# PM25/Information-Retrieval-with-Contrastive-Learning

Hardware: AMD Instinct MI355X
Metric: query-doc pairs/sec (train) + queries/sec @ top-k over N docs, 1/2/4/8 GPU (higher is better)
Workload: dtype bf16

## Files before the change

include/irc.h:

```cpp
#ifndef IRC_H_
#define IRC_H_

#include <stdint.h>

#ifdef __cplusplus
extern "C" {
#endif

typedef void* irc_stream_t;

#define IRC_OK 0
#define IRC_E_INVALID 1001
#define IRC_E_WORKSPACE 1002
#define IRC_E_LAUNCH 1003

const char* irc_last_error(void);
int irc_abi_version(void);

int64_t irc_scan_topk_workspace(int64_t Q, int64_t N, int64_t D, int64_t k);
int irc_scan_topk(const void* queries, const void* docs, int64_t Q, int64_t N, int64_t D,
                  int64_t k, int64_t doc_offset, void* workspace, int64_t workspace_bytes,
                  float* out_score, int64_t* out_idx, irc_stream_t stream);

int irc_scan_topk_many(const void* const* queries, int64_t batches, const void* docs, int64_t Q,
// ... 61 lines not shown
int irc_quantize_fp8(int in_dtype, const void* x, int64_t n, float scale, void* out,
                     irc_stream_t stream);

int irc_gemm(int in_dtype, int out_dtype, int a_layout, int b_layout, int epilogue, int64_t M,
             int64_t N, int64_t K, float alpha, const void* A, int64_t lda, int64_t strideA,
             const void* B, int64_t ldb, int64_t strideB, const float* bias, int64_t strideBias,
             const void* R, int64_t ldr, int64_t strideR, void* C, int64_t ldc, int64_t strideC,
             int accumulate, int64_t batch, void* workspace, int64_t workspace_bytes,
             irc_stream_t stream);
int64_t irc_gemm_workspace(int in_dtype, int out_dtype, int epilogue, int64_t M, int64_t N,
                           int64_t K, int64_t batch);
int irc_gemm_ex(int in_dtype, int out_dtype, int a_layout, int b_layout, int epilogue, int64_t M,
                int64_t N, int64_t K, float alpha, const void* A, int64_t lda, int64_t strideA,
                const void* B, int64_t ldb, int64_t strideB, const float* bias, int64_t strideBias,
                const void* R, int64_t ldr, int64_t strideR, void* C, int64_t ldc, int64_t strideC,
                int accumulate, int64_t batch, void* workspace, int64_t workspace_bytes,
                int64_t max_blocks, irc_stream_t stream);
int64_t irc_gemm_workspace_ex(int in_dtype, int out_dtype, int epilogue, int64_t M, int64_t N,
                              int64_t K, int64_t batch, int64_t max_blocks);
int irc_gemm_set_persistent(int mode);
int irc_gemm_set_big_ring(int on);
int irc_gemm_ln(int epilogue, int64_t M, int64_t N, int64_t K, const void* A, int64_t lda,
                const void* B, int64_t ldb, const float* bias, const void* R, int64_t ldr,
                void* C, int64_t ldc, const float* ln_stats, int ln_nt, const float* ln_gamma,
                const float* ln_beta, float ln_eps, int64_t ln_h, const float* fold_colsum,
                float* stats_out, int* stats_nt_out, irc_stream_t stream);
int irc_gemm_set_big_mf16(int on);
int irc_gemm_set_big_dma(int on);
int irc_gemm_big_dma_fits(int64_t M, int64_t N, int64_t K, int64_t lda, int64_t ldb);
int irc_gemm_set_l2_touch(int mode);
int64_t irc_gemm_l2_touch_map(int operand, int64_t tiles_m, int64_t tiles_n, int64_t window,
                              int64_t lines, int64_t nk, int64_t dist, int32_t* count,
                              int32_t* owner, int32_t* sharers);

int irc_gemm_set_pp(int on);

int irc_embed_ln(int dtype, const int64_t* ids, const void* word, const void* pos,
                 const void* type0, const float* gamma, const float* beta, void* y, int64_t rows,
                 int64_t L, int64_t H, float eps, irc_stream_t stream);
int irc_layernorm(int dtype, const void* x, void* y, const float* gamma, const float* beta,
                  int64_t rows, int64_t H, float eps, irc_stream_t stream);
int irc_attention(int dtype, const void* qkv, const int64_t* mask, void* ctx, int64_t B,
                  int64_t L, int64_t H, int64_t heads, irc_stream_t stream);
int irc_qkv_attention(int64_t M, int64_t H, int64_t heads, int64_t L, const void* x, int64_t ldx,
                      const void* wqkv_perm, const float* bias_perm, const int64_t* mask,
                      void* ctx, int64_t ldc, irc_stream_t stream);

int64_t irc_layernorm_bwd_workspace(int64_t rows, int64_t H);
int irc_layernorm_bwd(int dtype, int dy_dtype, const void* dy, const void* x, const float* gamma,
                      void* dx, float* dgamma, float* dbeta, float* partial,
                      int64_t partial_floats, int64_t rows, int64_t H, float eps, int64_t bcast_L,
                      float dy_scale, int accumulate, irc_stream_t stream);
int irc_attention_bwd(int dtype, const void* qkv, const int64_t* mask, const void* ctx,
                      const void* dctx, void* dqkv, int64_t B, int64_t L, int64_t H,
                      int64_t heads, irc_stream_t stream);
int irc_embed_sum(int dtype, const int64_t* ids, const void* word, const void* pos,
                  const void* type0, float* y, int64_t rows, int64_t L, int64_t H,
                  irc_stream_t stream);
int irc_embed_bwd(int dtype, const void* dx, const int64_t* ids, float* dword, float* dpos,
                  float* dtype0, float* workspace, int64_t ws_floats, int64_t B, int64_t L,
                  int64_t H, int64_t pad_id, irc_stream_t stream);

int irc_lstm_fwd(int dtype, const float* xp, const void* whh, void* hout, float* gsave,
                 float* csave, void* hprev, int64_t B, int64_t L, int64_t H, int64_t ndir,
                 irc_stream_t stream);
int irc_lstm_bwd(int dtype, const float* dy, const void* whh, const float* gsave,
// ... 159 lines not shown
```

information-retrieval-with-contrastive-learning_amd/csrc/gemm.hip:

```cpp
#include "gemm_epi.h"
#include "gemm_pp.h"

#include <algorithm>
#include <atomic>
#include <type_traits>

#ifndef IRC_GEMM_GROUP_M
#define IRC_GEMM_GROUP_M 0
#endif

namespace irc {
namespace gemm {

enum Layout { ROW = 0, COL = 1 };

constexpr int BM = 128, BN = 128, NT = 256;

template <typename T>
struct TT;
template <>
struct TT<unsigned short> {
  static constexpr int BK = 32;
  static constexpr int VEC = 8;
  static constexpr int PITCH = BK * 2 + 16;
// ... 424 lines not shown
  constexpr int CH = ROWS * 4;
  static_assert(CH % NT == 0, "whole passes");
#pragma unroll
  for (int i = 0; i < CH / NT; ++i) {
    const int p = (i * NW + wave) * 64 + lane;
    const int row = p >> 2;
    const int c = (p & 3) ^ ((row >> 2) & 3);
    int gr = r0 + row;
    gr = gr < nrows ? gr : nrows - 1;
    glds16(X + (int64_t)gr * ld + k0 + c * 8, lds_tile + (i * NW + wave) * 1024);
  }
}

#ifdef IRC_BIG_STAMPS
__device__ uint64_t big_stamps[64][5][2];
#define BSTAMP(kt, i)                                                                      \
  do {                                                                                     \
    __builtin_amdgcn_sched_barrier(0);                                                     \
    if (blockIdx.x == 0 && threadIdx.x == 0 && (kt) < 64) {                               \
      uint64_t c_, r_;                                                                     \
      asm volatile("s_memtime %0\n\ts_memrealtime %1\n\ts_waitcnt lgkmcnt(0)"            \
                   : "=s"(c_), "=s"(r_)::"memory");                                        \
      *(volatile uint64_t*)&big_stamps[(kt)][(i)][0] = c_;                                 \
      *(volatile uint64_t*)&big_stamps[(kt)][(i)][1] = r_;                                 \
    }                                                                                      \
    __builtin_amdgcn_sched_barrier(0);                                                     \
  } while (0)
#else
#define BSTAMP(kt, i) \
  do {                \
  } while (0)
#endif

template <int WNB>
__device__ __forceinline__ void mainloop_mf16(const unsigned short* A, int64_t lda,
                                              const unsigned short* B, int64_t ldb, int m0,
                                              int n0, int M, int N, int K, char* lds, int wave,
                                              int lane, f32x4 (&acc4)[8][2 * WNB], bool dma,
                                              const Touch tch, int ls = 0, int sh = 6) {
  constexpr int BN = 128 * WNB;
  constexpr int A_BYTES = BM * ROW_BYTES, STAGE = A_BYTES + BN * ROW_BYTES;
  const int wm = wave >> 2, wn = wave & 3;
  const int nk = K / BK;
  const int a_rows = ls == 0 ? 64 : ls;
  const int a_row0 = ls == 0 ? m0 : (m0 >> sh) * ls;
  const bool buf = dma && (ls == 0 || sh == 6) && a_row0 + (BM / 64) * a_rows <= M && n0 + BN <= N;
  const __amdgpu_buffer_rsrc_t ra = buffer_rsrc(A, (uint32_t)(((int64_t)(M - 1) * lda + K) * 2));
  const __amdgpu_buffer_rsrc_t rb = buffer_rsrc(B, (uint32_t)(((int64_t)(N - 1) * ldb + K) * 2));
  const uint32_t a_pass = (uint32_t)a_rows * (uint32_t)lda * 2u, b_pass = 128u * (uint32_t)ldb;
  const uint32_t a_tile = (uint32_t)a_row0 * (uint32_t)lda * 2u;
  const uint32_t b_tile = (uint32_t)n0 * (uint32_t)ldb * 2u;
  uint32_t a_lane = 0, b_lane = 0;
  uint32_t ta_lane = 0, tb_lane = 0, sink = 0;
  uint64_t ta_mask = 0, tb_mask = 0;
  int touch_nk = 0;
  if (buf && (tch.a_n | tch.b_n) != 0) {
    touch_nk = nk - TOUCH_D;
    const int t = wave * 64 + lane;
    const int ar = tch.a_lo + t;
    const int arow = ls == 0 ? ar : (ar >> 6) * ls + min(ar & 63, ls - 1);
    ta_lane = (uint32_t)arow * (uint32_t)lda * 2u;
    tb_lane = (uint32_t)(tch.b_lo + t) * (uint32_t)ldb * 2u;
    ta_mask = __builtin_amdgcn_ballot_w64(t < tch.a_n);
    tb_mask = __builtin_amdgcn_ballot_w64(t < tch.b_n);
  }
  if (buf) {
    a_lane = dma_lane_off(lda, wave, lane, ls);
// ... 18 lines not shown
    BSTAMP(kt, 0);
    char* nxt = lds + (cur ^ 1) * STAGE;
    if (more && buf) {
      const uint32_t kb = (uint32_t)(kt + 1) * ROW_BYTES;
      stage_buf<BM>(ra, a_lane, a_tile + kb, a_pass, nxt, wave);
      stage_buf<BN>(rb, b_lane, b_tile + kb, b_pass, nxt + A_BYTES, wave);
      if (kt < touch_nk) {
        const uint32_t kd = (uint32_t)(kt + TOUCH_D) * ROW_BYTES;
        if (ta_mask != 0) touch_dword(sink, ra, ta_lane, a_tile + kd, ta_mask);
        if (tb_mask != 0) touch_dword(sink, rb, tb_lane, b_tile + kd, tb_mask);
      }
    } else if (more) {
      int ln = lane;
      asm volatile("" : "+v"(ln));
      stage<BM>(A, lda, m0, M, (kt + 1) * BK, nxt, wave, ln, ls, sh);
      stage<BN>(B, ldb, n0, N, (kt + 1) * BK, nxt + A_BYTES, wave, ln);
    }
    BSTAMP(kt, 1);
    const char* la = lds + cur * STAGE;
    const char* lb = la + A_BYTES;
#pragma unroll
    for (int s2 = 0; s2 < 2; ++s2) {
      const int coff = (((4 * s2 + q4) ^ key) * 16);
      bf16x8 fa[8];
#pragma unroll
      for (int i = 0; i < 8; ++i)
        fa[i] = *reinterpret_cast<const bf16x8*>(la + (wm * 128 + i * 16 + l16) * 128 + coff);
#pragma unroll
      for (int j = 0; j < 2 * WNB; ++j) {
        const bf16x8 fb =
            *reinterpret_cast<const bf16x8*>(lb + (wn * 32 * WNB + j * 16 + l16) * 128 + coff);
#pragma unroll
        for (int i = 0; i < 8; ++i)
          acc4[i][j] = __builtin_amdgcn_mfma_f32_16x16x32_bf16(fa[i], fb, acc4[i][j], 0, 0, 0);
      }
    }
    BSTAMP(kt, 2);
    wait_vmcnt<0>();
    BSTAMP(kt, 3);
    __syncthreads();
    BSTAMP(kt, 4);
  }
  touch_done(sink);
}
}

inline std::atomic<int>& big_ring_mode() {
  static std::atomic<int> on{0};
  return on;
}
inline bool big_ring() { return big_ring_mode().load(std::memory_order_relaxed) != 0; }

inline std::atomic<int>& big_mf16_mode() {
  static std::atomic<int> on{1};
  return on;
}
inline bool big_mf16() { return big_mf16_mode().load(std::memory_order_relaxed) != 0; }

inline std::atomic<int>& big_dma_mode() {
  static std::atomic<int> on{1};
  return on;
}
inline int big_dma_flag(int64_t M, int64_t N, int64_t K, int64_t lda, int64_t ldb) {
  return big_dma_mode().load(std::memory_order_relaxed) != 0 && big::dma_fits(M, K, lda) &&
         big::dma_fits(N, K, ldb);
}

constexpr int L2_TOUCH_MAX_TILES_N = 2;
inline std::atomic<int>& l2_touch_mode() {
  static std::atomic<int> mode{[] {
    const char* e = getenv("IRC_GEMM_L2_TOUCH");
    return e && e[0] >= '0' && e[0] <= '2' ? e[0] - '0' : 1;
  }()};
  return mode;
}
inline int l2_touch_flag(int big_dma, int group_m, int64_t tiles_n) {
  const int mode = l2_touch_mode().load(std::memory_order_relaxed);
  if (mode == 0 || !big_dma || group_m > 1) return 0;
  if (mode == 1 && tiles_n > L2_TOUCH_MAX_TILES_N) return 0;
  const int cus = gpp::cu_count();
  return cus >= 8 ? cus / 8 : 32;
}

template <int EPI, int WNB>
__device__ __forceinline__ void big_epilogue_bf16(const Args& g, const f32x4 (&acc4)[8][2 * WNB],
                                                  char* lds, unsigned short* C,
                                                  const unsigned short* R, const float* bias,
                                                  int m0, int n0, int wave, int lane) {
  constexpr int BN = 128 * WNB, WCOLS = 32 * WNB, PITCH = WCOLS + 8;
  constexpr int CPR = WCOLS / 8;
  constexpr int NCH = 32 * CPR / 64;
  constexpr int NB = CPR == 12 ? 3 : 1;
  constexpr int RSTEP = 64 * NB / CPR;
  static_assert(64 * NB % CPR == 0 && NCH % NB == 0, "the chunk map repeats every NB iterations");
  constexpr bool READS_R = EPI == EPI_BIAS_RESID || EPI == EPI_RESID || EPI == EPI_DGELU;
  constexpr bool USES_R = READS_R || EPI == EPI_BIAS_GELU_SAVE;
  const int wm = wave >> 2, wn = wave & 3;
  float* st = reinterpret_cast<float*>(lds) + wave * (32 * PITCH);
// ... 98 lines not shown
        if constexpr (READS_R) {
          if (i < 3) load_r(i + 1, it);
        }
      }
    } else {
#pragma unroll
      for (int it = 0; it < NCH; ++it) {
        const int c = it * 64 + lane;
        const int rl = c / CPR, c8 = (c % CPR) * 8;
        const int row = rbase + rl, col = cbase + c8;
        if (row >= g.M || col >= g.N) continue;
        const f32x4 v0 = *reinterpret_cast<const f32x4*>(&st[rl * PITCH + c8]);
        const f32x4 v1 = *reinterpret_cast<const f32x4*>(&st[rl * PITCH + c8 + 4]);
        const unsigned short* rp = USES_R ? R + (int64_t)row * g.ldr + col : nullptr;
        u16x8 rr = {};
        if constexpr (READS_R) rr = *reinterpret_cast<const u16x8*>(rp);
        const u16x8 o = finish(v0, v1, rr, rp);
#ifdef IRC_PP_DIAG_NOSTORE
        if (o[0] == 0x7fc1 && o[7] == 0x7fc3)
#endif
        *reinterpret_cast<u16x8*>(C + (int64_t)row * g.ldc + col) = o;
      }
    }
    __builtin_amdgcn_wave_barrier();
    asm volatile("s_waitcnt lgkmcnt(0)" ::: "memory");
  }
  };
  if (fast)
    passes(std::true_type{});
  else
    passes(std::false_type{});
}

template <typename TO, int EPI, int WNB, bool RING = false, bool MF16 = false, bool LN = false>
__global__ __launch_bounds__(big::NT, 1) void gemm_big_kernel(Args g) {
  static_assert(!(RING && MF16), "the 16x16x32 form is 2-slot only");
  static_assert(!LN || (MF16 && sizeof(TO) == 2), "the LayerNorm fold: 16x16x32 form, bf16 C");
  using big::BK;
  using big::NT;
  using big::NW;
  constexpr int BM = big::BM, BN = 128 * WNB;
  constexpr int A_BYTES = BM * big::ROW_BYTES, B_BYTES = BN * big::ROW_BYTES;
  constexpr int STAGE = A_BYTES + B_BYTES;
  __shared__ __attribute__((aligned(1024))) char lds[2 * STAGE];
  const int tiles_m = (g.M + BM - 1) / BM;
  const int tiles_n = (g.N + BN - 1) / BN;
  const int ntiles = tiles_m * tiles_n;
  int bid = blockIdx.x;
  {
    const int q = ntiles / 8, r = ntiles % 8, x = bid % 8;
    bid = (x < r ? x * (q + 1) : r * (q + 1) + (x - r) * q) + bid / 8;
  }
  int tm, tn;
  grouped_tile(bid, tiles_m, tiles_n, g.group_m, tm, tn);
  const int batch = blockIdx.y;
  const unsigned short* A = reinterpret_cast<const unsigned short*>(g.A) + batch * g.sA;
  const unsigned short* B = reinterpret_cast<const unsigned short*>(g.B) + batch * g.sB;
  TO* C = reinterpret_cast<TO*>(g.C) + batch * g.sC;
  const int m0 = tm * BM, n0 = tn * BN;
  const int lane = threadIdx.x & 63;
  const int wave = __builtin_amdgcn_readfirstlane(threadIdx.x >> 6);
  const int wm = wave >> 2, wn = wave & 3;
  const int h = lane >> 5, r32 = lane & 31;

  f32x16 acc[4][WNB];
  f32x4 acc4[8][2 * WNB];
#pragma unroll
  for (int i = 0; i < 4; ++i)
#pragma unroll
    for (int j = 0; j < WNB; ++j) acc[i][j] = (f32x16)0.0f;
// ... 18 lines not shown
    const int sw4 = (r32 >> 2) & 3;
    for (int kt = 0; kt < nk; ++kt) {
      const int after = nk - 1 - kt;
      if (after >= 2) wait_vmcnt<2 * PPT>();
      else if (after == 1) wait_vmcnt<PPT>();
      else wait_vmcnt<0>();
      wg_barrier();
      if (kt + 3 < nk) {
        char* nxt = lds + ((kt + 3) & 3) * STG4;
        big::stage4<BM>(A, g.lda, m0, g.M, (kt + 3) * BK4, nxt, wave, lane);
        big::stage4<BN>(B, g.ldb, n0, g.N, (kt + 3) * BK4, nxt + A4, wave, lane);
      }
      const char* la = lds + (kt & 3) * STG4;
      const char* lb = la + A4;
#pragma unroll
      for (int kk = 0; kk < BK4 / 16; ++kk) {
        const int coff = ((2 * kk + h) ^ sw4) * 16;
        bf16x8 fa[4], fb[WNB];
#pragma unroll
        for (int i = 0; i < 4; ++i)
          fa[i] = *reinterpret_cast<const bf16x8*>(la + (wm * 128 + i * 32 + r32) * ROW4 + coff);
#pragma unroll
        for (int j = 0; j < WNB; ++j)
          fb[j] = *reinterpret_cast<const bf16x8*>(lb + (wn * 32 * WNB + j * 32 + r32) * ROW4 + coff);
#pragma unroll
        for (int i = 0; i < 4; ++i)
#pragma unroll
          for (int j = 0; j < WNB; ++j)
            acc[i][j] = __builtin_amdgcn_mfma_f32_32x32x16_bf16(fa[i], fb[j], acc[i][j], 0, 0, 0);
      }
    }
    __syncthreads();
  } else if constexpr (MF16) {
    big::mainloop_mf16<WNB>(A, g.lda, B, g.ldb, m0, n0, g.M, g.N, g.K, lds, wave, lane, acc4,
                            g.big_dma != 0,
                            big::touch_lines(g.l2_touch, tiles_m, tiles_n, tm, tn, BM, BN));
  } else {
  const int nk = g.K / BK;
  big::stage<BM>(A, g.lda, m0, g.M, 0, lds, wave, lane);
  big::stage<BN>(B, g.ldb, n0, g.N, 0, lds + A_BYTES, wave, lane);
  wait_vmcnt<0>();
  __syncthreads();
  const int swz = big::chunk_key(r32);
  for (int kt = 0; kt < nk; ++kt) {
    const int cur = kt & 1;
#ifdef IRC_PP_DIAG_NODMA
    const bool more = kt + 1 < nk && kt < 0;
#else
    const bool more = kt + 1 < nk;
#endif
    if (more) {
      char* nxt = lds + (cur ^ 1) * STAGE;
      big::stage<BM>(A, g.lda, m0, g.M, (kt + 1) * BK, nxt, wave, lane);
      big::stage<BN>(B, g.ldb, n0, g.N, (kt + 1) * BK, nxt + A_BYTES, wave, lane);
    }
    const char* la = lds + cur * STAGE;
    const char* lb = la + A_BYTES;
#pragma unroll
    for (int kk = 0; kk < BK / 16; ++kk) {
      const int coff = (((2 * kk + h) ^ swz) * 16);
      bf16x8 fa[4], fb[WNB];
#pragma unroll
      for (int i = 0; i < 4; ++i)
        fa[i] = *reinterpret_cast<const bf16x8*>(la + (wm * 128 + i * 32 + r32) * 128 + coff);
#pragma unroll
      for (int j = 0; j < WNB; ++j)
        fb[j] = *reinterpret_cast<const bf16x8*>(lb + (wn * 32 * WNB + j * 32 + r32) * 128 + coff);
#pragma unroll
      for (int i = 0; i < 4; ++i)
// ... 567 lines not shown
          for (int e = 0; e < 16; ++e) {
            const int i = 32 * ib + (e & 3) + 8 * (e >> 2) + 4 * h;
            if (i < g.L) out[(int64_t)i * g.ldc + 32 * db + r32] = f32_to_bf16(o[db][e]);
          }
      }
    }
    if (hf == 0) __syncthreads();
  }
}

inline int big_wnb(const Args& g, int batch, int la, int lb) {
  if (la != ROW || lb != ROW || !g.vec_a || !g.vec_b) return 0;
  if (g.K % big::BK != 0 || g.K == 0) return 0;
  const int wnb = g.N % 384 == 0 ? 3 : 2;
  const int64_t tiles = (int64_t)((g.M + 255) / 256) * ((g.N + 128 * wnb - 1) / (128 * wnb)) * batch;
  return tiles >= 128 ? wnb : 0;
}

template <typename TO, int EPI, bool LN = false>
static int launch_big(const Args& g0, int batch, int wnb, hipStream_t st) {
  Args g = g0;
  g.big_dma = big_dma_flag(g.M, g.N, g.K, g.lda, g.ldb);
  const int bn = 128 * wnb;
  g.l2_touch = l2_touch_flag(g.big_dma, g.group_m, (g.N + bn - 1) / bn);
  const int tiles = ((g.M + big::BM - 1) / big::BM) * ((g.N + bn - 1) / bn);
  prof_begin(st);
  const bool ring = big_ring() && g.K % big::BK4 == 0;
  if constexpr (LN) {
    if (wnb == 3)
      hipLaunchKernelGGL((gemm_big_kernel<TO, EPI, 3, false, true, true>), dim3(tiles, batch), dim3(big::NT), 0, st, g);
    else
      hipLaunchKernelGGL((gemm_big_kernel<TO, EPI, 2, false, true, true>), dim3(tiles, batch), dim3(big::NT), 0, st, g);
  } else if (big_mf16() && !ring) {
    if (wnb == 3)
      hipLaunchKernelGGL((gemm_big_kernel<TO, EPI, 3, false, true>), dim3(tiles, batch), dim3(big::NT), 0, st, g);
    else
      hipLaunchKernelGGL((gemm_big_kernel<TO, EPI, 2, false, true>), dim3(tiles, batch), dim3(big::NT), 0, st, g);
  } else if (wnb == 3 && ring)
    hipLaunchKernelGGL((gemm_big_kernel<TO, EPI, 3, true>), dim3(tiles, batch), dim3(big::NT), 0, st, g);
  else if (wnb == 3)
    hipLaunchKernelGGL((gemm_big_kernel<TO, EPI, 3>), dim3(tiles, batch), dim3(big::NT), 0, st, g);
  else if (ring)
    hipLaunchKernelGGL((gemm_big_kernel<TO, EPI, 2, true>), dim3(tiles, batch), dim3(big::NT), 0, st, g);
  else
    hipLaunchKernelGGL((gemm_big_kernel<TO, EPI, 2>), dim3(tiles, batch), dim3(big::NT), 0, st, g);
  prof_end("gemm_bf16", st, 2.0 * g.M * g.N * g.K * batch);
  prof_work("gemm_bf16_bytes", gemm_alg_bytes(sizeof(TO) == 4, EPI, g.accumulate, g.M, g.N, g.K,
                                               batch));
  return check_launch("gemm_big_kernel");
}

template <typename TI, typename TO, int LA, int LB, int EPI>
static int launch(const Args& g0, int batch, int splits, hipStream_t st) {
  if constexpr (sizeof(TI) == 2) {
    if (splits == 1) {
      const int wnb = big_wnb(g0, batch, LA, LB);
      if (wnb) return launch_big<TO, EPI>(g0, batch, wnb, st);
    }
  }
  Args g = g0;
  const int tiles = ((g.M + BM - 1) / BM) * ((g.N + BN - 1) / BN);
  constexpr int bk = TT<TI>::BK;
  g.kchunk = splits > 1 ? ((g.K + splits - 1) / splits + bk - 1) / bk * bk : (g.K > 0 ? g.K : 1);
  prof_begin(st);
  hipLaunchKernelGGL((gemm_kernel<TI, TO, LA, LB, EPI>), dim3(tiles, batch, splits), dim3(NT), 0,
                     st, g);
  if (splits > 1) {
// ... 201 lines not shown
extern "C" int64_t irc_gemm_l2_touch_map(int operand, int64_t tiles_m, int64_t tiles_n,
                                         int64_t window, int64_t lines, int64_t nk,
                                         int64_t dist, int32_t* count, int32_t* owner,
                                         int32_t* sharers) {
  using namespace irc::gemm;
  if ((operand != 0 && operand != 1) || tiles_m < 1 || tiles_n < 1 || window < 1 || lines < 1 ||
      lines > big::NT || nk < 1 || dist < 1 || tiles_m > (1 << 20) || tiles_n > (1 << 20) ||
      window > (1 << 20) || !count || !owner)
    return -1;
  for (int64_t i = 0; i < nk * lines; ++i) count[i] = 0, owner[i] = -1;
  int s_a, rank_a, s_b, rank_b;
  big::touch_share((int)tiles_m, (int)tiles_n, (int)window, 0, 0, s_a, rank_a, s_b, rank_b);
  const int s = operand == 0 ? s_a : s_b;
  if (sharers) *sharers = s;
  int64_t outside = 0;
  for (int rank = 0; rank < s; ++rank) {
    const big::Touch t = big::touch_lines((int)window, (int)tiles_m, (int)tiles_n,
                                          operand == 0 ? 0 : rank, operand == 0 ? rank : 0,
                                          (int)lines, (int)lines);
    const int lo = operand == 0 ? t.a_lo : t.b_lo, n = operand == 0 ? t.a_n : t.b_n;
    for (int64_t kt = 0; kt + dist < nk; ++kt)
      for (int th = 0; th < big::NT; ++th) {
        if (th >= n) continue;
        const int64_t k = kt + dist, r = lo + th;
        if (r < 0 || r >= lines || k >= nk) {
          ++outside;
          continue;
        }
        ++count[k * lines + r];
        owner[k * lines + r] = rank;
      }
  }
  return outside;
}

extern "C" int irc_gemm_set_big_ring(int on) {
  return irc::gemm::big_ring_mode().exchange(on ? 1 : 0);
}

extern "C" int irc_gemm_ex(int in_dtype, int out_dtype, int a_layout, int b_layout, int epilogue,
                           int64_t M, int64_t N, int64_t K, float alpha, const void* A, int64_t lda,
                           int64_t strideA, const void* B, int64_t ldb, int64_t strideB,
                           const float* bias, int64_t strideBias, const void* R, int64_t ldr,
                           int64_t strideR, void* C, int64_t ldc, int64_t strideC, int accumulate,
                           int64_t batch, void* workspace, int64_t workspace_bytes,
                           int64_t max_blocks, irc_stream_t stream) {
  const int64_t bud = split_budget(max_blocks);
  IRC_REQUIRE(M >= 0 && N >= 0 && K >= 0 && batch >= 1, "gemm: bad sizes");
  IRC_REQUIRE(M < (1ll << 31) && N < (1ll << 31) && K < (1ll << 31), "gemm: size too large");
  IRC_REQUIRE(in_dtype == 0 || in_dtype == 1, "gemm: in_dtype must be 0 (bf16) or 1 (fp32)");
  IRC_REQUIRE(out_dtype == 0 || out_dtype == 1, "gemm: out_dtype must be 0 (bf16) or 1 (fp32)");
  IRC_REQUIRE(!(accumulate && out_dtype == 0), "gemm: accumulate needs fp32 C");
  IRC_REQUIRE(epilogue >= 0 && epilogue <= 6, "gemm: bad epilogue");
  IRC_REQUIRE(!gemm::epi_has_bias(epilogue) || bias, "gemm: epilogue needs bias");
  IRC_REQUIRE(!(epilogue >= 3 && epilogue != 1 && epilogue != 2) || R,
              "gemm: epilogue needs R (residual / pre-activation)");
  IRC_REQUIRE(!(accumulate && epilogue >= 5), "gemm: accumulate with a GELU epilogue");
  const int vec = in_dtype == 0 ? 8 : 4;
  const int vec_a = lda % vec == 0 && strideA % vec == 0 && ((uintptr_t)A % 16) == 0;
  const int vec_b = ldb % vec == 0 && strideB % vec == 0 && ((uintptr_t)B % 16) == 0;
  if (M == 0 || N == 0) return IRC_OK;
  int splits = gemm::split_count(in_dtype == 0 ? 2 : 4, out_dtype == 1, epilogue, M, N, K, batch, bud);
  if (splits > 1 && (workspace == nullptr ||
                     workspace_bytes < (int64_t)splits * M * N * batch * (int64_t)sizeof(float)))
    splits = 1;
  const int cvec = out_dtype == 0 ? 8 : 4;
// ... 59 lines not shown
```

information-retrieval-with-contrastive-learning_amd/irc_amd/_lib.py:

```python
from __future__ import annotations

import ctypes
import os
import threading

_HERE = os.path.dirname(os.path.abspath(__file__))
LIB_PATH = os.path.join(_HERE, "lib", "libirc_hip.so")
LIB_PATH = os.environ.get("IRC_LIB_PATH") or LIB_PATH

_c = ctypes
P = _c.c_void_p
I64 = _c.c_int64
I32 = _c.c_int
U32 = _c.c_uint32
F32 = _c.c_float

SIGNATURES = {
    "irc_last_error": (_c.c_char_p, []),
    "irc_abi_version": (I32, []),
    "irc_scan_topk_workspace": (I64, [I64, I64, I64, I64]),
    "irc_scan_topk": (I32, [P, P, I64, I64, I64, I64, I64, P, I64, P, P, P]),
    "irc_scan_topk_many": (I32, [P, I64, P, I64, I64, I64, I64, I64, P, I64, I64, P, P, P, P]),
    "irc_corpus_pack": (I32, [P, P, I64, I64, P, P, P]),
    "irc_pair_sample": (I32, [P, P, P, P, I64, P, P]),
# ... 15 lines not shown
    "irc_rerank_topk_stream_fp8": (I32, [P, P, I64, I64, I64, P, P, I64, I64, I64, F32, P, I64, P,
                                         P, P, P]),
    "irc_rerank_topk_grouped_workspace": (I64, [I64, I64, I64]),
    "irc_rerank_topk_grouped": (I32, [P, P, I64, I64, I64, P, P, I64, I64, I64, P, I64, U32, F32,
                                      P, I64, P, P, P, P]),
    "irc_scan_topk_fp8_workspace": (I64, [I64, I64, I64, I64]),
    "irc_scan_topk_fp8": (I32, [P, P, I64, I64, I64, I64, I64, F32, P, I64, P, P, P]),
    "irc_scan_scores_fp8": (I32, [P, P, I64, I64, I64, P, P]),
    "irc_quantize_fp8": (I32, [I32, P, I64, F32, P, P]),
    "irc_csr_union_chunks": (I64, [I64]),
    "irc_csr_union_count": (I32, [P, P, I64, P, P, I64, I64, P, P, P]),
    "irc_csr_union_emit": (I32, [P, I64, I64, P, P, P, P]),
    "irc_csr_spmv_f64": (I32, [P, P, P, I64, P, P, P, I64, P, P]),
    "irc_topk_f64": (I32, [P, I64, P, P, I64, I64, P, P, P, P]),
    "irc_proto_ce": (I32, [P, P, I64, I64, P, P, P, P]),
    "irc_argmax_bias": (I32, [P, P, I64, I64, P, P, P]),
    "irc_centroid_accumulate": (I32, [P, P, I64, I64, P, P, P]),
    "irc_centroid_finalize": (I32, [P, P, I64, I64, P, P, P]),
    "irc_gemm": (I32, [I32, I32, I32, I32, I32, I64, I64, I64, F32, P, I64, I64, P, I64, I64,
                       P, I64, P, I64, I64, P, I64, I64, I32, I64, P, I64, P]),
    "irc_gemm_workspace": (I64, [I32, I32, I32, I64, I64, I64, I64]),
    "irc_gemm_ex": (I32, [I32, I32, I32, I32, I32, I64, I64, I64, F32, P, I64, I64, P, I64, I64,
                          P, I64, P, I64, I64, P, I64, I64, I32, I64, P, I64, I64, P]),
    "irc_gemm_workspace_ex": (I64, [I32, I32, I32, I64, I64, I64, I64, I64]),
    "irc_gemm_set_persistent": (I32, [I32]),
    "irc_gemm_set_big_ring": (I32, [I32]),
    "irc_gemm_ln": (I32, [I32, I64, I64, I64, P, I64, P, I64, P, P, I64, P, I64, P, I32, P, P, F32,
                          I64, P, P, P, P]),
    "irc_gemm_set_big_mf16": (I32, [I32]),
    "irc_gemm_set_big_dma": (I32, [I32]),
    "irc_gemm_big_dma_fits": (I32, [I64, I64, I64, I64, I64]),
    "irc_gemm_set_l2_touch": (I32, [I32]),
    "irc_gemm_l2_touch_map": (I64, [I32, I64, I64, I64, I64, I64, I64, P, P, P]),
    "irc_gemm_set_pp": (I32, [I32]),
    "irc_scan_set_ppl_min_q": (I32, [I32]),
    "irc_embed_ln": (I32, [I32, P, P, P, P, P, P, P, I64, I64, I64, F32, P]),
    "irc_layernorm": (I32, [I32, P, P, P, P, I64, I64, F32, P]),
    "irc_attention": (I32, [I32, P, P, P, I64, I64, I64, I64, P]),
    "irc_qkv_attention": (I32, [I64, I64, I64, I64, P, I64, P, P, P, P, I64, P]),
    "irc_layernorm_bwd_workspace": (I64, [I64, I64]),
    "irc_layernorm_bwd": (I32, [I32, I32, P, P, P, P, P, P, P, I64, I64, I64, F32, I64, F32, I32,
                                P]),
    "irc_attention_bwd": (I32, [I32, P, P, P, P, P, I64, I64, I64, I64, P]),
    "irc_embed_sum": (I32, [I32, P, P, P, P, P, I64, I64, I64, P]),
    "irc_embed_bwd": (I32, [I32, P, P, P, P, P, P, I64, I64, I64, I64, I64, P]),
    "irc_lstm_fwd": (I32, [I32, P, P, P, P, P, P, I64, I64, I64, I64, P]),
    "irc_lstm_bwd": (I32, [I32, P, P, P, P, P, I64, I64, I64, I64, P]),
    "irc_lstm_mfma_supported": (I32, [I64]),
    "irc_lstm_mfma_save_floats": (I64, [I64, I64, I64, I64, I32]),
    "irc_lstm_pack": (I32, [P, P, P, P, I64, I64, I64, P, P, P, P, P]),
    "irc_lstm_fwd_mfma": (I32, [P, P, P, P, P, P, I64, I64, I64, I64, P]),
    "irc_lstm_bwd_mfma": (I32, [P, P, P, P, P, I64, I64, I64, I64, P]),
    "irc_lstm_hprev": (I32, [P, P, I64, I64, I64, I64, P]),
    "irc_lstm_coop_supported": (I32, [I64]),
    "irc_lstm_coop_sizes": (I64, [I64, I64, I64, I64, I32]),
    "irc_lstm_coop_pack": (I32, [P, I64, I64, P, P, P]),
    "irc_lstm_fwd_coop": (I32, [P, P, P, P, P, P, P, P, I64, I64, I64, I64, P]),
    "irc_lstm_bwd_coop": (I32, [P, P, P, P, P, P, P, I64, I64, I64, I64, P]),
    "irc_lstm_coop_fault": (I32, [P, I64, I64, P, P]),
    "irc_mean_rows": (I32, [I32, P, P, I64, I64, I64, I64, P]),
    "irc_bcast_rows": (I32, [P, P, I64, I64, I64, F32, P]),
    "irc_l2norm_fwd": (I32, [P, P, P, I64, I64, F32, P]),
    "irc_l2norm_bwd": (I32, [P, P, P, P, I64, I64, F32, P]),
    "irc_nce_lse": (I32, [P, P, I64, I64, F32, P, P, P]),
    "irc_nce_grads": (I32, [P, P, P, I64, I64, F32, P, P, P, P]),
    "irc_axpby": (I32, [P, P, P, F32, F32, I64, P]),
# ... 76 lines not shown
```

information-retrieval-with-contrastive-learning_amd/irc_amd/ops.py:

```python
from __future__ import annotations

import ctypes

import torch

from . import _lib
from ._lib import IRCError
from ._torch import ptr, require_hip, stream_ptr

BF16, F32 = torch.bfloat16, torch.float32
_DT = {BF16: 0, F32: 1}

EPI_NONE, EPI_BIAS, EPI_BIAS_GELU, EPI_BIAS_RESID, EPI_RESID = 0, 1, 2, 3, 4


def _code(t: torch.Tensor) -> int:
    try:
        return _DT[t.dtype]
    except KeyError:
        raise TypeError(f"irc kernels take bf16 or fp32, got {t.dtype}") from None


def gemm_set_big_ring(on) -> int:
    return int(_lib.load().irc_gemm_set_big_ring(1 if on else 0))
# ... 45 lines not shown
    return out


def gemm_set_big_mf16(on) -> int:
    return int(_lib.load().irc_gemm_set_big_mf16(1 if on else 0))


def gemm_set_big_dma(on) -> int:
    return int(_lib.load().irc_gemm_set_big_dma(1 if on else 0))


def gemm_big_dma_fits(M, N, K, lda, ldb) -> bool:
    return bool(_lib.load().irc_gemm_big_dma_fits(M, N, K, lda, ldb))


def gemm_set_l2_touch(mode) -> int:
    return int(_lib.load().irc_gemm_set_l2_touch(int(mode)))


def gemm_l2_touch_map(operand, tiles_m, tiles_n, window, lines, nk, dist):
    import numpy as np

    count = np.empty((nk, lines), dtype=np.int32)
    owner = np.empty((nk, lines), dtype=np.int32)
    sharers = ctypes.c_int(0)
    outside = _lib.load().irc_gemm_l2_touch_map(
        int(operand), tiles_m, tiles_n, window, lines, nk, dist, count.ctypes.data,
        owner.ctypes.data, ctypes.addressof(sharers))
    if outside < 0:
        raise ValueError("gemm_l2_touch_map: bad arguments")
    return count, owner, int(sharers.value), int(outside)


def gemm_set_pp(on) -> int:
    return int(_lib.load().irc_gemm_set_pp(1 if on else 0))


def gemm_set_persistent(mode) -> int:
    return int(_lib.load().irc_gemm_set_persistent(int(mode)))


def gemm(a, b, *, trans_a=False, b_is_nk=True, bias=None, epilogue=EPI_NONE, residual=None,
         alpha=1.0, out=None, out_dtype=None, accumulate=False, max_blocks=0):
    require_hip(a, b, bias, residual, out)
    if a.dtype != b.dtype:
        raise TypeError(f"gemm operands must share a dtype ({a.dtype} vs {b.dtype})")
    if a.stride(-1) != 1 or b.stride(-1) != 1:
        raise ValueError("gemm operands must be contiguous in their last dim")
    M, K = (a.shape[1], a.shape[0]) if trans_a else (a.shape[0], a.shape[1])
    N, Kb = (b.shape[0], b.shape[1]) if b_is_nk else (b.shape[1], b.shape[0])
    if K != Kb:
        raise ValueError(f"gemm inner dims differ: {K} vs {Kb}")
    if out is None:
        od = out_dtype or a.dtype
        out = torch.empty((M, N), dtype=od, device=a.device)
        if accumulate:
            out.zero_()
    if bias is not None and bias.dtype != F32:
        raise TypeError("bias must be fp32")
    if residual is not None and residual.dtype != out.dtype:
        raise TypeError("residual dtype must match the output")
    ws, nws = _splitk_ws(a, out, epilogue, M, N, K, 1, max_blocks)
    _lib.call("irc_gemm_ex", _code(a), _code(out), 1 if trans_a else 0, 0 if b_is_nk else 1,
              int(epilogue), M, N, K, float(alpha), ptr(a), a.stride(0), 0, ptr(b), b.stride(0),
              0, ptr(bias), 0, ptr(residual), residual.stride(0) if residual is not None else 0, 0,
              ptr(out), out.stride(0), 0, 1 if accumulate else 0, 1, ptr(ws), nws,
# ... 564 lines not shown
```

Before: 34710.

## Add direct-to-global bf16 epilogue for big MF16 GEMM with swapped MFMA operands

Adds a DIRECT variant of the big 16x16x32 GEMM kernel. It swaps the MFMA operands so the accumulators are transposed, then writes bias/GELU epilogue results straight to global memory as 16-byte vector stores, using permlane16 swaps to regroup lanes. The old epilogue path is skipped for interior tiles. The aim is to remove the LDS staging round trip and its barriers at the end of each tile. It is on by default for bias and bias+GELU. Bias+residual needs mode 2 and reads the residual with a small prefetch. It adds new kernel instantiations, a store-map debug export and alignment preconditions.

```diff
diff --git a/include/irc.h b/include/irc.h
--- a/include/irc.h
+++ b/include/irc.h
@@ -117,6 +117,8 @@
 int64_t irc_gemm_l2_touch_map(int operand, int64_t tiles_m, int64_t tiles_n, int64_t window,
                               int64_t lines, int64_t nk, int64_t dist, int32_t* count,
                               int32_t* owner, int32_t* sharers);
+int irc_gemm_set_big_direct(int mode);
+int irc_gemm_direct_store_map(int wnb, int32_t* row, int32_t* col);
 
 int irc_gemm_set_pp(int on);
 
diff --git a/information-retrieval-with-contrastive-learning_amd/csrc/gemm.hip b/information-retrieval-with-contrastive-learning_amd/csrc/gemm.hip
--- a/information-retrieval-with-contrastive-learning_amd/csrc/gemm.hip
+++ b/information-retrieval-with-contrastive-learning_amd/csrc/gemm.hip
@@ -480,7 +480,7 @@
   } while (0)
 #endif
 
-template <int WNB>
+template <int WNB, bool SWAP = false>
 __device__ __forceinline__ void mainloop_mf16(const unsigned short* A, int64_t lda,
                                               const unsigned short* B, int64_t ldb, int m0,
                                               int n0, int M, int N, int K, char* lds, int wave,
@@ -565,7 +565,8 @@
             *reinterpret_cast<const bf16x8*>(lb + (wn * 32 * WNB + j * 16 + l16) * 128 + coff);
 #pragma unroll
         for (int i = 0; i < 8; ++i)
-          acc4[i][j] = __builtin_amdgcn_mfma_f32_16x16x32_bf16(fa[i], fb, acc4[i][j], 0, 0, 0);
+          acc4[i][j] = SWAP ? __builtin_amdgcn_mfma_f32_16x16x32_bf16(fb, fa[i], acc4[i][j], 0, 0, 0)
+                            : __builtin_amdgcn_mfma_f32_16x16x32_bf16(fa[i], fb, acc4[i][j], 0, 0, 0);
       }
     }
     BSTAMP(kt, 2);
@@ -576,6 +577,14 @@
   }
   touch_done(sink);
 }
+
+constexpr int DIRECT_ROW_BLOCKS = 8;
+__host__ __device__ inline void direct_piece(int wnb, int wave, int lane, int s, int& row,
+                                             int& col) {
+  const int wm = wave >> 2, wn = wave & 3, q = lane >> 4;
+  row = 128 * wm + 16 * (s / wnb) + (lane & 15);
+  col = 32 * wnb * wn + 32 * (s % wnb) + 16 * (q & 1) + 8 * (q >> 1);
+}
 }
 
 inline std::atomic<int>& big_ring_mode() {
@@ -597,6 +606,16 @@
 inline int big_dma_flag(int64_t M, int64_t N, int64_t K, int64_t lda, int64_t ldb) {
   return big_dma_mode().load(std::memory_order_relaxed) != 0 && big::dma_fits(M, K, lda) &&
          big::dma_fits(N, K, ldb);
+}
+
+inline std::atomic<int>& big_direct_mode() {
+  static std::atomic<int> on{1};
+  return on;
+}
+inline bool big_direct_flag(int epi, const void* bias, int64_t stride_bias) {
+  const int mode = big_direct_mode().load(std::memory_order_relaxed);
+  if (mode == 0 || (mode == 1 && epi == EPI_BIAS_RESID)) return false;
+  return bias != nullptr && (uintptr_t)bias % 16 == 0 && stride_bias % 4 == 0;
 }
 
 constexpr int L2_TOUCH_MAX_TILES_N = 2;
@@ -761,10 +780,93 @@
     passes(std::false_type{});
 }
 
-template <typename TO, int EPI, int WNB, bool RING = false, bool MF16 = false, bool LN = false>
+constexpr bool epi_direct(int e) {
+  return e == EPI_BIAS || e == EPI_BIAS_GELU || e == EPI_BIAS_RESID;
+}
+__device__ __forceinline__ void swap16(uint32_t& a, uint32_t& b) {
+#ifdef __HIP_DEVICE_COMPILE__
+  const auto r = __builtin_amdgcn_permlane16_swap(a, b, false, false);
+  a = r[0];
+  b = r[1];
+#endif
+}
+template <int EPI, int WNB>
+__device__ __forceinline__ void big_epilogue_direct(const Args& g, const f32x4 (&acc4)[8][2 * WNB],
+                                                    unsigned short* C, const unsigned short* R,
+                                                    const float* bias, int m0, int n0, int wave,
+                                                    int lane) {
+  static_assert(epi_direct(EPI), "bias, bias + GELU, bias + residual");
+  constexpr bool READS_R = EPI == EPI_BIAS_RESID;
+  constexpr int R_AHEAD = 2;
+  typedef uint32_t u32x4 __attribute__((ext_vector_type(4)));
+  typedef __bf16 bf16x2 __attribute__((ext_vector_type(2)));
+  int lrow, lcol, wrow, wcol;
+  big::direct_piece(WNB, wave & 3, lane, 0, lrow, lcol);
+  big::direct_piece(WNB, wave & 4, 0, 0, wrow, wcol);
+  const uint32_t coff = 2u * (uint32_t)(lrow * (int)g.ldc + lcol);
+  const uint32_t roff = READS_R ? 2u * (uint32_t)(lrow * (int)g.ldr + lcol) : 0u;
+  f32x4 bv[2 * WNB];
+#pragma unroll
+  for (int j = 0; j < 2 * WNB; ++j)
+    bv[j] = *reinterpret_cast<const f32x4*>(bias + n0 + 32 * WNB * (wave & 3) + 16 * j +
+                                            4 * (lane >> 4));
+  const f32x2_t alpha = {g.alpha, g.alpha};
+  u32x4 rq[R_AHEAD][WNB];
+  auto load_r = [&](int i, int jp) {
+    int row, col;
+    big::direct_piece(WNB, 0, 0, i * WNB + jp, row, col);
+    const char* ru = reinterpret_cast<const char*>(R + (int64_t)(m0 + wrow + row) * g.ldr + n0);
+    rq[i % R_AHEAD][jp] = *reinterpret_cast<const u32x4*>(ru + 2 * col + roff);
+  };
+  if constexpr (READS_R) {
+#pragma unroll
+    for (int i = 0; i < R_AHEAD; ++i)
+#pragma unroll
+      for (int jp = 0; jp < WNB; ++jp) load_r(i, jp);
+  }
+#pragma unroll
+  for (int i = 0; i < big::DIRECT_ROW_BLOCKS; ++i)
+#pragma unroll
+    for (int jp = 0; jp < WNB; ++jp) {
+      uint32_t rr[2][2] = {{0, 0}, {0, 0}}, pk[2][2];
+      if constexpr (READS_R) {
+        const u32x4 r4 = rq[i % R_AHEAD][jp];
+        rr[0][0] = r4[0], rr[0][1] = r4[1], rr[1][0] = r4[2], rr[1][1] = r4[3];
+        swap16(rr[0][0], rr[1][0]);
+        swap16(rr[0][1], rr[1][1]);
+        if (i + R_AHEAD < big::DIRECT_ROW_BLOCKS) load_r(i + R_AHEAD, jp);
+      }
+#pragma unroll
+      for (int b = 0; b < 2; ++b)
+#pragma unroll
+        for (int e = 0; e < 4; e += 2) {
+          const int j = 2 * jp + b;
+          const f32x4& a = acc4[i][j];
+          f32x2_t v = __builtin_elementwise_fma(f32x2_t{a[e], a[e + 1]}, alpha,
+                                                f32x2_t{bv[j][e], bv[j][e + 1]});
+          if constexpr (EPI == EPI_BIAS_GELU) v = gelu_lite2(v);
+          if constexpr (READS_R) {
+            v.x = v.x + bf16_to_f32((unsigned short)(rr[b][e / 2] & 0xffffu));
+            v.y = v.y + bf16_to_f32((unsigned short)(rr[b][e / 2] >> 16));
+          }
+          pk[b][e / 2] = __builtin_bit_cast(uint32_t, __builtin_convertvector(v, bf16x2));
+        }
+      swap16(pk[0][0], pk[1][0]);
+      swap16(pk[0][1], pk[1][1]);
+      int row, col;
+      big::direct_piece(WNB, 0, 0, i * WNB + jp, row, col);
+      char* cu = reinterpret_cast<char*>(C + (int64_t)(m0 + wrow + row) * g.ldc + n0);
+      *reinterpret_cast<u32x4*>(cu + 2 * col + coff) = u32x4{pk[0][0], pk[0][1], pk[1][0], pk[1][1]};
+    }
+}
+
+template <typename TO, int EPI, int WNB, bool RING = false, bool MF16 = false, bool LN = false,
+          bool DIRECT = false>
 __global__ __launch_bounds__(big::NT, 1) void gemm_big_kernel(Args g) {
   static_assert(!(RING && MF16), "the 16x16x32 form is 2-slot only");
   static_assert(!LN || (MF16 && sizeof(TO) == 2), "the LayerNorm fold: 16x16x32 form, bf16 C");
+  static_assert(!DIRECT || (MF16 && !LN && sizeof(TO) == 2 && epi_direct(EPI)),
+                "the direct epilogue: 16x16x32 form, bf16 C, epilogues 1 / 2 / 3");
   using big::BK;
   using big::NT;
   using big::NW;
@@ -849,9 +951,22 @@
     }
     __syncthreads();
   } else if constexpr (MF16) {
+    const big::Touch tch = big::touch_lines(g.l2_touch, tiles_m, tiles_n, tm, tn, BM, BN);
+    if constexpr (DIRECT) {
+      const bool interior = g.vec_c && m0 + BM <= g.M && n0 + BN <= g.N && g.ldc < (1 << 24) &&
+                            (EPI != EPI_BIAS_RESID || g.ldr < (1 << 24));
+      if (interior) {
+        big::mainloop_mf16<WNB, true>(A, g.lda, B, g.ldb, m0, n0, g.M, g.N, g.K, lds, wave, lane,
+                                      acc4, g.big_dma != 0, tch);
+        big_epilogue_direct<EPI, WNB>(
+            g, acc4, reinterpret_cast<unsigned short*>(C),
+            g.R ? reinterpret_cast<const unsigned short*>(g.R) + batch * g.sR : nullptr,
+            g.bias + batch * g.sBias, m0, n0, wave, lane);
+        return;
+      }
+    }
     big::mainloop_mf16<WNB>(A, g.lda, B, g.ldb, m0, n0, g.M, g.N, g.K, lds, wave, lane, acc4,
-                            g.big_dma != 0,
-                            big::touch_lines(g.l2_touch, tiles_m, tiles_n, tm, tn, BM, BN));
+                            g.big_dma != 0, tch);
   } else {
   const int nk = g.K / BK;
   big::stage<BM>(A, g.lda, m0, g.M, 0, lds, wave, lane);
@@ -1485,7 +1600,13 @@
     else
       hipLaunchKernelGGL((gemm_big_kernel<TO, EPI, 2, false, true, true>), dim3(tiles, batch), dim3(big::NT), 0, st, g);
   } else if (big_mf16() && !ring) {
-    if (wnb == 3)
+    constexpr bool CAN = sizeof(TO) == 2 && epi_direct(EPI);
+    const bool direct = CAN && big_direct_flag(EPI, g.bias, g.sBias);
+    if (direct && wnb == 3)
+      hipLaunchKernelGGL((gemm_big_kernel<TO, EPI, 3, false, true, false, CAN>), dim3(tiles, batch), dim3(big::NT), 0, st, g);
+    else if (direct)
+      hipLaunchKernelGGL((gemm_big_kernel<TO, EPI, 2, false, true, false, CAN>), dim3(tiles, batch), dim3(big::NT), 0, st, g);
+    else if (wnb == 3)
       hipLaunchKernelGGL((gemm_big_kernel<TO, EPI, 3, false, true>), dim3(tiles, batch), dim3(big::NT), 0, st, g);
     else
       hipLaunchKernelGGL((gemm_big_kernel<TO, EPI, 2, false, true>), dim3(tiles, batch), dim3(big::NT), 0, st, g);
@@ -1753,6 +1874,28 @@
       }
   }
   return outside;
+}
+
+extern "C" int irc_gemm_set_big_direct(int mode) {
+  return irc::gemm::big_direct_mode().exchange(mode < 0 ? 0 : mode > 2 ? 2 : mode);
+}
+
+extern "C" int irc_gemm_direct_store_map(int wnb, int32_t* row, int32_t* col) {
+  using namespace irc::gemm;
+  if ((wnb != 2 && wnb != 3) || !row || !col) return -1;
+  const int ns = big::DIRECT_ROW_BLOCKS * wnb;
+  for (int wave = 0; wave < big::NW; ++wave)
+    for (int lane = 0; lane < 64; ++lane)
+      for (int s = 0; s < ns; ++s) {
+        int lrow, lcol, wrow, wcol, srow, scol;
+        big::direct_piece(wnb, wave & 3, lane, 0, lrow, lcol);
+        big::direct_piece(wnb, wave & 4, 0, 0, wrow, wcol);
+        big::direct_piece(wnb, 0, 0, s, srow, scol);
+        const int at = (wave * 64 + lane) * ns + s;
+        row[at] = wrow + srow + lrow;
+        col[at] = wcol + scol + lcol;
+      }
+  return ns;
 }
 
 extern "C" int irc_gemm_set_big_ring(int on) {
diff --git a/information-retrieval-with-contrastive-learning_amd/irc_amd/_lib.py b/information-retrieval-with-contrastive-learning_amd/irc_amd/_lib.py
--- a/information-retrieval-with-contrastive-learning_amd/irc_amd/_lib.py
+++ b/information-retrieval-with-contrastive-learning_amd/irc_amd/_lib.py
@@ -71,6 +71,8 @@
     "irc_gemm_big_dma_fits": (I32, [I64, I64, I64, I64, I64]),
     "irc_gemm_set_l2_touch": (I32, [I32]),
     "irc_gemm_l2_touch_map": (I64, [I32, I64, I64, I64, I64, I64, I64, P, P, P]),
+    "irc_gemm_set_big_direct": (I32, [I32]),
+    "irc_gemm_direct_store_map": (I32, [I32, P, P]),
     "irc_gemm_set_pp": (I32, [I32]),
     "irc_scan_set_ppl_min_q": (I32, [I32]),
     "irc_embed_ln": (I32, [I32, P, P, P, P, P, P, P, I64, I64, I64, F32, P]),
diff --git a/information-retrieval-with-contrastive-learning_amd/irc_amd/ops.py b/information-retrieval-with-contrastive-learning_amd/irc_amd/ops.py
--- a/information-retrieval-with-contrastive-learning_amd/irc_amd/ops.py
+++ b/information-retrieval-with-contrastive-learning_amd/irc_amd/ops.py
@@ -101,6 +101,21 @@
     return count, owner, int(sharers.value), int(outside)
 
 
+def gemm_set_big_direct(mode) -> int:
+    return int(_lib.load().irc_gemm_set_big_direct(int(mode)))
+
+
+def gemm_direct_store_map(wnb):
+    import numpy as np
+
+    row = np.full((8, 64, 8 * max(int(wnb), 0)), -1, dtype=np.int32)
+    col = np.full_like(row, -1)
+    n = _lib.load().irc_gemm_direct_store_map(int(wnb), row.ctypes.data, col.ctypes.data)
+    if n != row.shape[2] or n <= 0:
+        raise ValueError("gemm_direct_store_map: wnb must be 2 or 3")
+    return row, col
+
+
 def gemm_set_pp(on) -> int:
     return int(_lib.load().irc_gemm_set_pp(1 if on else 0))
 
```

Result: no change. 34890, median of 6 (+0.5%).
